# 3dlg-hcvc/tricolo

Hardware: AMD Instinct MI355X
Metric: trimodal training samples/sec (32^3 voxel + 6-view) (higher is better)
Workload: dtype f16 (f16 activation storage + f16 MFMA operands, fp32 accumulate; bf16x3 heads/GRU; within 1e-3 of the fp32 reference)

## Files before the change

### include/tricolo_hip.h

```cpp
#ifndef TRICOLO_HIP_H
#define TRICOLO_HIP_H
#include <stddef.h>
#include <stdint.h>

#ifdef __cplusplus
extern "C" {
#endif

#define TRI_FMT_F32 0
#define TRI_FMT_BF16 1
#define TRI_FMT_F16 2

int tri_version(void);
const char* tri_last_error(void);

typedef struct TriConvDesc {
    int B, ID, IH, IW, Cin;
    int OD, OH, OW, Cout;
    int KD, KH, KW, stride, pad_d, pad_h, pad_w;
} TriConvDesc;

int tri_conv_kpad(int ntaps, int cin_stored);
typedef struct TriPrepDesc {
    const float* w;
// ... 16 lines not shown
int tri_linear_small_supported(int M, int K, int N);
int tri_linear_small_fwd(const float* x, const float* w, const float* bias, float* y, int M, int K, int N, int act, int split3, void* stream);
int tri_linear_small_dgrad(const float* dout, const float* y, const float* w, float* dx, int M, int K, int N, int act, int split3,
                           void* stream);
int tri_linear_small_wgrad(const float* x, const float* dout, const float* y, float* dw, float* db , int M, int K, int N,
                           int act, int split3, void* stream);
int tri_linear_small_bwd(const float* x, const float* dout, const float* y, const float* w, float* dx, float* dw, float* db, int M, int K,
                         int N, int act, int split3, void* stream);

int tri_conv_num_mtiles(const TriConvDesc* d, int split3);
int tri_conv_num_records(const TriConvDesc* d, int split3, int row_list);
int tri_conv_kernel_family(const TriConvDesc* d, int transposed, int split3);
int tri_conv_wgrad_kernel_family(const TriConvDesc* d, int act_fmt);
size_t tri_conv_workspace(const TriConvDesc* d, int transposed);
int tri_conv_fwd(const TriConvDesc* d, const void* in, const void* w_hi, const void* w_lo, void* out, const uint8_t* row_mask,
                 const float* bias, int act, int accumulate, float* stats, int act_fmt, void* workspace, size_t workspace_bytes,
                 const int* row_pos , const int* row_count ,
                 void* stream);
int tri_conv_dgrad(const TriConvDesc* d, const void* dout, const void* wt_hi, const void* wt_lo, void* din, const uint8_t* row_mask,
                   int accumulate, int act_fmt, void* workspace, size_t workspace_bytes,
                   const int* row_pos ,
                   const int* row_count ,
                   void* stream);
typedef struct TriConvBnSums {
    const void* y;
    const float* relu_scale;
    const float* relu_shift;
    const void* relu_out;
    float* partial;
} TriConvBnSums;
int tri_conv_dgrad_bn_records(const TriConvDesc* d, int accumulate, int act_fmt);
int tri_conv_dgrad_bn(const TriConvDesc* d, const void* dout, const void* wt_hi, const void* wt_lo, void* din, int accumulate,
                      int act_fmt, void* workspace, size_t workspace_bytes, const int* row_pos, const TriConvBnSums* sums, void* stream);
size_t tri_conv_wgrad_workspace(const TriConvDesc* d);
size_t tri_conv_plan_bytes(const TriConvDesc* d);
int tri_conv_plan_build(const TriConvDesc* d, void* plan, void* stream);
int tri_conv_wgrad(const TriConvDesc* d, const void* in, const void* dout, const uint8_t* row_mask, const void* plan ,
                   void* workspace, size_t workspace_bytes, float* dw, long s_co, long s_tap, long s_ci, int cin_real, int split3,
                   int act_fmt, float out_scale ,
                   const int* row_pos, const int* row_count ,
                   void* stream);
#ifndef TRI_WGRAD_GROUP_MAX
#define TRI_WGRAD_GROUP_MAX 24
#endif
typedef struct TriWgradReduce {
    const float* slab;
    float* dw;
    long s_co, s_tap, s_ci;
    int splits, Cout, Kpad, ntaps, cin_stored, cin_real, zlanes, nblocks;
    float out_scale;
    int kw_real;
    int kw_shift;
} TriWgradReduce;
int tri_conv_wgrad_partial(const TriConvDesc* d, const void* in, const void* dout, const uint8_t* row_mask, const void* plan ,
                           void* workspace, size_t workspace_bytes, float* dw, long s_co, long s_tap, long s_ci, int cin_real, int split3,
                           int act_fmt, float out_scale, const int* row_pos, const int* row_count, TriWgradReduce* pending ,
                           void* stream);
int tri_wgrad_reduce_grouped(const TriWgradReduce* pending , int n, void* stream);
int tri_wgrad_reduce_grouped_noted(const TriWgradReduce* pending , int n, int* note, void* stream);
#define TRI_WGRAD_JOBS_MAX 12
typedef struct TriWgradJob {
    const TriConvDesc* d;
    const void* in;
    const void* dout;
    const void* plan;
    void* workspace;
// ... 181 lines not shown
```

### tricolo_amd/_C.py

```python
from __future__ import annotations

import ctypes as C
import os

import torch

_HERE = os.path.dirname(os.path.abspath(__file__))
LIB_PATH = os.path.join(_HERE, "libtricolo_hip.so")


class TriConvDesc(C.Structure):
    _fields_ = [(n, C.c_int) for n in ("B", "ID", "IH", "IW", "Cin", "OD", "OH", "OW", "Cout",
                                       "KD", "KH", "KW", "stride", "pad_d", "pad_h", "pad_w")]


class TriPrepDesc(C.Structure):
    _fields_ = [("w", C.c_void_p), ("hi", C.c_void_p), ("lo", C.c_void_p), ("s_row", C.c_long), ("s_tap", C.c_long),
                ("s_inner", C.c_long), ("rows", C.c_int), ("ntaps", C.c_int), ("inner", C.c_int), ("inner_pad", C.c_int),
                ("kpad", C.c_int), ("fmt", C.c_int), ("frag", C.c_int)]


class TriWgradReduce(C.Structure):
    _fields_ = [("slab", C.c_void_p), ("dw", C.c_void_p), ("s_co", C.c_long), ("s_tap", C.c_long), ("s_ci", C.c_long)] + \
               [(n, C.c_int) for n in ("splits", "Cout", "Kpad", "ntaps", "cin_stored", "cin_real", "zlanes", "nblocks")] + \
# ... 9 lines not shown
class TriConvBnSums(C.Structure):
    _fields_ = [("y", C.c_void_p), ("relu_scale", C.c_void_p), ("relu_shift", C.c_void_p), ("relu_out", C.c_void_p), ("partial", C.c_void_p)]


TRI_WGRAD_JOBS_MAX = 12
TRI_ERR_ARG, TRI_ERR_UNSUPPORTED = -1, -2

P, I, L, F, Z, DBL = C.c_void_p, C.c_int, C.c_long, C.c_float, C.c_size_t, C.c_double
DP = C.POINTER(TriConvDesc)

SIGNATURES = {
    "tri_version": (I, []),
    "tri_last_error": (C.c_char_p, []),
    "tri_conv_kpad": (I, [I, I]),
    "tri_weight_prep": (I, [P, L, L, L, I, I, I, I, P, P, I, I, P]),
    "tri_weight_prep_multi": (I, [P, I, P]),
    "tri_embedding_fwd": (I, [P, P, I, I, I, P, P]),
    "tri_embedding_bwd": (I, [P, P, I, I, I, I, I, P, P]),
    "tri_retrieval_topk": (I, [P, P, P, I, I, I, I, P, P, P, P]),
    "tri_linear_small_supported": (I, [I, I, I]),
    "tri_linear_small_fwd": (I, [P, P, P, P, I, I, I, I, I, P]),
    "tri_linear_small_dgrad": (I, [P, P, P, P, I, I, I, I, I, P]),
    "tri_linear_small_wgrad": (I, [P, P, P, P, P, I, I, I, I, I, P]),
    "tri_linear_small_bwd": (I, [P, P, P, P, P, P, P, I, I, I, I, I, P]),
    "tri_conv_num_mtiles": (I, [DP, I]),
    "tri_conv_num_records": (I, [DP, I, I]),
    "tri_conv_workspace": (Z, [DP, I]),
    "tri_conv_kernel_family": (I, [DP, I, I]),
    "tri_conv_wgrad_kernel_family": (I, [DP, I]),
    "tri_conv_fwd": (I, [DP, P, P, P, P, P, P, I, I, P, I, P, Z, P, P, P]),
    "tri_conv_dgrad": (I, [DP, P, P, P, P, P, I, I, P, Z, P, P, P]),
    "tri_conv_dgrad_bn_records": (I, [DP, I, I]),
    "tri_conv_dgrad_bn": (I, [DP, P, P, P, P, I, I, P, Z, P, C.POINTER(TriConvBnSums), P]),
    "tri_conv_wgrad_workspace": (Z, [DP]),
    "tri_conv_plan_bytes": (Z, [DP]),
    "tri_conv_plan_build": (I, [DP, P, P]),
    "tri_conv_wgrad": (I, [DP, P, P, P, P, P, Z, P, L, L, L, I, I, I, F, P, P, P]),
    "tri_conv_wgrad_partial": (I, [DP, P, P, P, P, P, Z, P, L, L, L, I, I, I, F, P, P, P, P]),
    "tri_wgrad_reduce_grouped": (I, [P, I, P]),
    "tri_wgrad_reduce_grouped_noted": (I, [P, I, P, P]),
    "tri_conv_stem_wgrad_bn": (I, [DP, P, P, P, P, P, P, P, P, P, P, Z, P, L, L, L, I, I, F, P, P]),
    "tri_conv_wgrad_group_info": (I, [DP, I, P, P, P]),
    "tri_conv_wgrad_partial_group": (I, [P, I, I, P, P]),
    "tri_bn_finalize": (I, [P, I, I, P, I, P, P, P, P, P, F, F, P, P, P, P, P]),
    "tri_bn_eval_coeffs": (I, [I, P, P, P, P, F, P, P, P, P, P]),
    "tri_bn_act": (I, [P, P, P, P, P, P, P, L, I, I, I, P]),
    "tri_relu_bwd": (I, [P, P, P, L, I, P]),
    "tri_bn_bwd_num_blocks": (I, [L]),
    "tri_bn_bwd_reduce": (I, [P, P, L, I, P, P, P, P, P, I, P]),
    "tri_bn_bwd_finalize": (I, [P, I, I, P, I, P, P, P, P, P, P, P, P, F, P]),
    "tri_bn_bwd_small": (I, [P, P, L, I, P, I, P, P, P, P, P, P, P, P, I, P, P, P, F, I, P]),
    "tri_bn_bwd_apply": (I, [P, P, P, P, P, P, P, L, I, P, P, P, P, I, I, P]),
    "tri_bn_bwd_pair_reduce": (I, [P, P, P, P, L, I, P, P, I, P]),
    "tri_bn_bwd_pair_finalize": (I, [P, P, I, I, I, P, P, P, P, P, P, P, P, F, P]),
    "tri_bn_bwd_pair_apply": (I, [P, P, P, P, P, P, P, P, P, L, I, I, P]),
    "tri_bn_relu_pool3d_fwd": (I, [P, P, P, P, I, I, I, P, P, I, P]),
    "tri_pool3d_bwd_route": (I, [P, P, P, P, P, P, I, I, I, P, I, P]),
    "tri_pool3d_bwd_route_rows": (I, [P, P, P, P, P, P, I, I, I, P, P, P, I, P]),
    "tri_pool3d_bwd_route_rows_num_blocks": (I, [I, I, I]),
    "tri_pool3d_bwd_route_rows_reduce": (I, [P, P, P, P, P, P, I, I, I, P, P, P, P, I, P]),
    "tri_bn_bwd_apply_rows": (I, [P, P, P, P, P, P, I, P, P, L, I, P]),
    "tri_bn_bwd_rows_scratch": (C.c_size_t, [I]),
    "tri_bn_bwd_rows": (I, [P, P, I, P, P, L, P, P, P, P, P, P, F, P, I, P]),
    "tri_pool3d_bwd_route_reduce_num_blocks": (I, [I, I, I]),
    "tri_pool3d_bwd_route_reduce": (I, [P, P, P, P, P, P, I, I, I, P, P, I, P]),
    "tri_maxpool2d_fwd": (I, [P, I, I, I, I, P, P, P, P, I, P]),
# ... 57 lines not shown
    "tri_adam_guard_segments": (I, [P, P, I, L, P, P]),
    "tri_adam_step": (I, [P, P, P, P, L, P, F, P, F, F, F, F, F, P]),
    "tri_adam_step_segments": (I, [P, P, P, I, P, P, L, P, F, P, F, F, F, F, F, P]),
}

_lib = None


def lib():
    global _lib
    if _lib is None:
        if not os.path.exists(LIB_PATH):
            raise ImportError(
                f"{LIB_PATH} not found: the HIP extension is not built.  Run `make -C tricolo_amd/csrc` "
                "(or __graft_entry__.build()).  tricolo_amd has no CPU fallback.")
        l = C.CDLL(LIB_PATH)
        for name, (res, args) in SIGNATURES.items():
            fn = getattr(l, name)
            fn.restype, fn.argtypes = res, args
        _lib = l
    return _lib


class _TimedLib:

    def __init__(self, real):
        self._real, self.records = real, []

    def __getattr__(self, name):
        fn = getattr(self._real, name)
        sig = SIGNATURES.get(name)
        if sig is None or not name.startswith("tri_") or not sig[1] or sig[0] is not I or name in ("tri_last_error",):
            return fn
        if "workspace" in name or "num_" in name or "_info" in name or "kpad" in name or "family" in name or "bytes" in name or "supported" in name or "scratch" in name or "records" in name:
            return fn

        shape_args = {"tri_bn_bwd_reduce": (2, 3), "tri_bn_bwd_apply": (7, 8), "tri_bn_act": (7, 8), "tri_bn_finalize": (1, 2),
                      "tri_bn_bwd_finalize": (1, 2), "tri_bn_bwd_small": (2, 3)}.get(name)

        def timed(*a):
            e0, e1 = torch.cuda.Event(enable_timing=True), torch.cuda.Event(enable_timing=True)
            e0.record()
            rc = fn(*a)
            e1.record()
            key = name if shape_args is None else f"{name}[{int(a[shape_args[0]])}x{int(a[shape_args[1]])}]"
            self.records.append((key, e0, e1))
            return rc
        return timed


def install_timing_proxy():
    global _lib
    real = lib()
    if isinstance(real, _TimedLib):
        return real
    _lib = _TimedLib(real)
    return _lib


def check(rc: int, what: str = ""):
    if rc != 0:
        msg = lib().tri_last_error().decode(errors="replace")
        raise RuntimeError(f"libtricolo_hip {what} failed (code {rc}): {msg}")


def ptr(t):
    if t is None:
# ... 13 lines not shown
```

### tricolo_amd/csrc/conv_igemm.hip

```cpp
#include "common.h"
#include <stdlib.h>
#include <map>
#include <mutex>
#include "../../include/tricolo_hip.h"
#include "conv_vox.h"

struct ConvArgs {
    const void* in;
    const void* w_hi;
    const void* w_lo;
    void* out;
    const uint8_t* row_mask;
    const int* row_pos;
    const int* row_count;
    const float* bias;
    float* stats;
    float* slab;
    int B, ID, IH, IW, Cin;
    int OD, OH, OW, Cout;
    int KD, KH, KW, stride, pd, ph, pw;
    int transposed, act, accumulate;
    int Kpad, M, ntaps, cin_shift, ksplit, steps_per_split;
    unsigned in_bytes;
    int nunits;
    int h_tr, h_rows, h_slab_bytes, h_nr, h_mtiles;
    int h_dbuf;
    int h_abl;
    int h_xcg, h_touch;
    int h_swz;
#ifdef HALO_STAMPS
    long long* h_dbg;
#endif
    FastDiv dOW, dOH, dOD, dCin, dP, dH2;
};

template <int N>
__device__ __forceinline__ float row_ror(float v) {
    return __builtin_bit_cast(float, __builtin_amdgcn_update_dpp(0, __builtin_bit_cast(int, v), 0x120 + N, 0xf, 0xf, false));
}

template <typename AT, int BN, int TM, int TN, int WAVES_M, int WM, int WN>
__device__ __forceinline__ void conv_epilogue(const ConvArgs& p, f32x4 (&acc)[TM][TN], int m0, int n0, int mtile, int wm, int wn, int fr,
                                              int fq, int t, int split, int any_active, float* red, int Meff) {
    if (p.ksplit > 1) {
// ... 282 lines not shown
            }
        };

        if (ks0 < ks1) {
            load_global(ks0);
            store_lds(0);
            __syncthreads();
            for (int ks = ks0; ks < ks1; ++ks) {
                const int buf = (ks - ks0) & 1;
                if (ks + 1 < ks1) load_global(ks + 1);
                compute(buf);
                if (ks + 1 < ks1) store_lds(buf ^ 1);
                __syncthreads();
            }
        }
    }

    conv_epilogue<AT, BN, TM, TN, WAVES_M, WM, WN>(p, acc, m0, n0, mtile, wm, wn, fr, fq, t, split, any_active, red, Meff);
}

__device__ __forceinline__ int dma_off(int row, int chunk) { return row * 128 + (((chunk ^ (row >> 1)) & 7) << 4); }

__device__ __forceinline__ void wait_vmcnt(int n) {
    switch (n) {
#define TRI_W(N) case N: asm volatile("s_waitcnt vmcnt(" #N ")" ::: "memory"); break;
        TRI_W(0) TRI_W(1) TRI_W(2) TRI_W(3) TRI_W(4) TRI_W(5) TRI_W(6) TRI_W(7) TRI_W(8) TRI_W(9) TRI_W(10) TRI_W(11) TRI_W(12)
        TRI_W(13) TRI_W(14) TRI_W(15) TRI_W(16) TRI_W(17) TRI_W(18) TRI_W(19) TRI_W(20) TRI_W(21) TRI_W(22) TRI_W(23) TRI_W(24)
        TRI_W(25) TRI_W(26) TRI_W(27) TRI_W(28) TRI_W(29) TRI_W(30) TRI_W(31) TRI_W(32)
#undef TRI_W
        default: asm volatile("s_waitcnt vmcnt(0)" ::: "memory"); break;
    }
}

template <int BN, int NST, typename AT>
__global__ __launch_bounds__(256) void conv_dma_kernel(const ConvArgs p) {
    typedef Mma<typename OpOf<AT>::E> MM;
    typedef typename MM::v8 v8;
    constexpr int BM = 128, BK = 64;
    constexpr int WAVES_N = 2, WAVES_M = 2;
    constexpr int WM = BM / WAVES_M, WN = BN / WAVES_N, TM = WM / 16, TN = WN / 16;
    constexpr int A_BYTES = BM * 128, B_BYTES = BN * 128, STAGE = A_BYTES + B_BYTES;
    extern __shared__ __attribute__((aligned(16))) char smem[];
    int* lut_off = (int*)(smem + NST * STAGE);
    int* lut_sh = lut_off + 64;
    float* red = (float*)(smem + NST * STAGE + 512);

    const int t = threadIdx.x, lane = t & 63, wave = t >> 6;
    const int NT = p.Cout / BN;
    const int wg = p.row_count ? (int)blockIdx.x : xcd_remap(blockIdx.x, gridDim.x);
    const int mtile = wg / NT, ntile = wg - mtile * NT;
    const int m0 = mtile * BM, n0 = ntile * BN;
    const int sshift = (p.stride == 2) ? 1 : 0;
    const int Meff = p.row_count ? min(*p.row_count, p.M) : p.M;
    if (m0 >= Meff) {
        if (p.stats && p.ksplit == 1 && t < BN) {
            p.stats[((size_t)mtile * 2 + 0) * p.Cout + n0 + t] = 0.f;
            p.stats[((size_t)mtile * 2 + 1) * p.Cout + n0 + t] = 0.f;
        }
        return;
    }

    if (t < 64) {
        int kd = 0, kh = 0, kw = 0;
        if (t < p.ntaps) {
            kw = t % p.KW;
            int r = t / p.KW;
            kh = r % p.KH;
// ... 43 lines not shown
        ax |= (unsigned)__builtin_amdgcn_update_dpp(0, (int)ax, 0x128, 0xf, 0xf, false);
        ax |= (unsigned)__builtin_amdgcn_update_dpp(0, (int)ax, 0x124, 0xf, 0xf, false);
        ax |= (unsigned)__builtin_amdgcn_update_dpp(0, (int)ax, 0x122, 0xf, 0xf, false);
        ax |= (unsigned)__builtin_amdgcn_update_dpp(0, (int)ax, 0x121, 0xf, 0xf, false);
        ax = (unsigned)(__builtin_amdgcn_readlane((int)ax, 0) | __builtin_amdgcn_readlane((int)ax, 16) |
                        __builtin_amdgcn_readlane((int)ax, 32) | __builtin_amdgcn_readlane((int)ax, 48));
        if (lane == 0) wave_axes[wave] = ax;
    }
    any_active = __syncthreads_or(any_active);

    f32x4 acc[TM][TN];
#pragma unroll
    for (int a = 0; a < TM; ++a)
#pragma unroll
        for (int b = 0; b < TN; ++b) acc[a][b] = (f32x4){0.f, 0.f, 0.f, 0.f};

    const int wm = wave / WAVES_N, wn = wave - wm * WAVES_N;
    const int fr = lane & 15, fq = lane >> 4;
    const int split = blockIdx.y;

    if (any_active) {
        const int nk_total = p.Kpad >> 6;
        const int ks0 = split * p.steps_per_split;
        const int ks1 = min(nk_total, ks0 + p.steps_per_split);
        const v4i rsrc = make_rsrc_words(p.in, p.in_bytes);
        const v4i wrsrc = make_rsrc_words((const uint16_t*)p.w_hi + (size_t)n0 * p.Kpad, (unsigned)(BN * p.Kpad * 2));
        const unsigned lds0 = lds_addr(smem) + wave * 1024;
        int woff[BN / 32];
#pragma unroll
        for (int i = 0; i < BN / 32; ++i) {
            int n = (t >> 3) + 32 * i;
            woff[i] = (n * p.Kpad + (slot ^ ((n >> 1) & 7)) * 8) * 2;
        }

        auto issue = [&](int ks, int buf) {
            const unsigned base = lds0 + buf * STAGE;
            const int kb = ks * BK;
            int tap, c0;
            if (p.cin_shift >= 0) { tap = kb >> p.cin_shift; c0 = kb & ((1 << p.cin_shift) - 1); }
            else { tap = (int)fdiv((uint32_t)kb, p.dCin); c0 = kb - tap * p.Cin; }
            const bool tv = tap < p.ntaps;
            const int toff = (lut_off[tv ? tap : 0] + c0) * 2;
            const int sh = lut_sh[tv ? tap : 0];
            const int sx = sh & 255, sy = (sh >> 8) & 255, sz = (sh >> 16) & 255;
#pragma unroll
            for (int i = 0; i < 4; ++i) {
                unsigned mk = rmask[i];
                bool ok = tv && (((mk >> sx) & (mk >> sy) & (mk >> sz)) & 1u);
                int voff = ok ? rowoff[i] + toff : (int)0x80000000;
                dma16_async(rsrc, base + i * 4096, voff);
            }
#pragma unroll
            for (int i = 0; i < BN / 32; ++i) {
                dma16_async(wrsrc, base + A_BYTES + i * 4096, woff[i] + kb * 2);
            }
        };
        auto compute = [&](int buf) {
            const char* base = smem + buf * STAGE;
            const char* bb = base + A_BYTES;
#pragma unroll
            for (int kk = 0; kk < 2; ++kk) {
                v8 ah[TM];
#pragma unroll
                for (int a = 0; a < TM; ++a) ah[a] = *(const v8*)(base + dma_off(wm * WM + a * 16 + fr, kk * 4 + fq));
#pragma unroll
                for (int b = 0; b < TN; ++b) {
                    v8 bhf = *(const v8*)(bb + dma_off(wn * WN + b * 16 + fr, kk * 4 + fq));
#pragma unroll
                    for (int a = 0; a < TM; ++a) acc[a][b] = MM::mma(bhf, ah[a], acc[a][b]);
                }
            }
        };

        int nl = ks1 - ks0;
        if (p.row_pos) {
            if (wave == 0) {
                const unsigned axes = wave_axes[0] | wave_axes[1] | wave_axes[2] | wave_axes[3];
                int count = 0;
                for (int base = 0; base < ks1 - ks0; base += 64) {
                    const int ks = ks0 + base + lane;
                    bool ok = false;
                    if (ks < ks1) {
                        const int kb = ks * BK;
                        const int tap = p.cin_shift >= 0 ? (kb >> p.cin_shift) : (int)fdiv((uint32_t)kb, p.dCin);
                        if (tap < p.ntaps) {
                            const int sh = lut_sh[tap];
                            ok = ((axes >> (sh & 255)) & (axes >> ((sh >> 8) & 255)) & (axes >> ((sh >> 16) & 255))) & 1u;
                        }
                    }
                    const unsigned long long bal = __ballot(ok);
                    if (ok && count + __popcll(bal & ((1ull << lane) - 1ull)) < 256)
                        live_steps[count + __popcll(bal & ((1ull << lane) - 1ull))] = ks;
                    count += __popcll(bal);
                }
                if (lane == 0) nlive_s = count;
            }
            __syncthreads();
            nl = nlive_s;
        }
        auto step_at = [&](int j) { return p.row_pos ? live_steps[j] : ks0 + j; };
        if (nl > 0) {
            constexpr int PER = 4 + BN / 32;
#pragma unroll
            for (int d = 0; d < NST - 1; ++d)
                if (d < nl) issue(step_at(d), d);
            int buf = 0;
            for (int j = 0; j < nl; ++j) {
                const int younger = min(nl - 1 - j, NST - 2);
                if (NST == 2 || younger == 0) wait_vmcnt(0);
                else if (younger == 1) wait_vmcnt(PER);
                else wait_vmcnt(2 * PER);
                __builtin_amdgcn_s_barrier();
                asm volatile("" ::: "memory");
                if (j + NST - 1 < nl) {
                    int nb = buf + NST - 1;
                    if (nb >= NST) nb -= NST;
                    issue(step_at(j + NST - 1), nb);
                }
                compute(buf);
                if (++buf == NST) buf = 0;
            }
        }
        __syncthreads();
    }
    conv_epilogue<AT, BN, TM, TN, WAVES_M, WM, WN>(p, acc, m0, n0, mtile, wm, wn, fr, fq, t, split, any_active, red, Meff);
// ... 1857 lines not shown
    return conv_dispatch(a, act_fmt, workspace, workspace_bytes, (hipStream_t)stream);
}

extern "C" int tri_conv_dgrad_bn_records(const TriConvDesc* d, int accumulate, int act_fmt) {
    (void)accumulate;
    if (act_fmt != TRI_FMT_BF16 && act_fmt != TRI_FMT_F16) return 0;
    ConvPlan pl = conv_make_plan(d->B, d->OD, d->OH, d->OW, d->Cout, d->ID, d->IH, d->IW, d->Cin, d->KD, d->KH, d->KW, d->stride, d->pad_d,
                                 d->pad_h, d->pad_w, 2, 0);
    if (pl.c64 && d->IW <= 32) return pl.c64_grid;
    return 0;
}
extern "C" int tri_conv_dgrad_bn(const TriConvDesc* d, const void* dout, const void* wt_hi, const void* wt_lo, void* din, int accumulate,
                                 int act_fmt, void* workspace, size_t workspace_bytes, const int* row_pos, const TriConvBnSums* sums,
                                 void* stream) {
    if (!sums || !sums->y || !sums->partial || (!sums->relu_scale != !sums->relu_shift) || (sums->relu_scale && sums->relu_out)) {
        tri_set_error("tri_conv_dgrad_bn: sums needs y, partial and at most one of (relu_scale + relu_shift) / relu_out");
        return TRI_ERR_ARG;
    }
    if (tri_conv_dgrad_bn_records(d, accumulate, act_fmt) == 0) {
        tri_set_error("tri_conv_dgrad_bn: no fused form for this layer (tri_conv_dgrad_bn_records == 0)");
        return TRI_ERR_UNSUPPORTED;
    }
    ConvArgs a{};
    a.in = dout; a.w_hi = wt_hi; a.w_lo = wt_lo; a.out = din;
    a.row_pos = row_pos;
    a.B = d->B; a.ID = d->OD; a.IH = d->OH; a.IW = d->OW; a.Cin = d->Cout;
    a.OD = d->ID; a.OH = d->IH; a.OW = d->IW; a.Cout = d->Cin;
    a.KD = d->KD; a.KH = d->KH; a.KW = d->KW; a.stride = d->stride; a.pd = d->pad_d; a.ph = d->pad_h; a.pw = d->pad_w;
    a.transposed = 1; a.act = 0; a.accumulate = accumulate;
    a.ntaps = d->KD * d->KH * d->KW;
    a.M = d->B * d->ID * d->IH * d->IW;
    return conv_dispatch(a, act_fmt, workspace, workspace_bytes, (hipStream_t)stream, sums);
}
```

### tricolo_amd/model/module/img_encoder/mv_cnn.py

```python
from __future__ import annotations

import os

import torch
import torch.nn as nn

from .... import ops
from ....layers import SideStream, TriModule, linear_bwd, linear_fwd, require_gpu


_DS_FWD = int(os.environ.get("TRICOLO_DS_FWD", "2"))
_DS_BWD = int(os.environ.get("TRICOLO_DS_BWD", "2"))
_PREP_DGRAD_LATE = os.environ.get("TRICOLO_PREP_DGRAD_LATE", "1") != "0"
_BN_PAIR = True
_STEM_BESIDE_WGRAD = os.environ.get("TRICOLO_STEM_BESIDE_WGRAD", "1") != "0"
_PREP_ISSUE = int(os.environ.get("TRICOLO_PREP_ISSUE", "1"))


class _BasicBlockParams(nn.Module):
    def __init__(self, inplanes, planes, stride):
        super().__init__()
        self.conv1 = nn.Conv2d(inplanes, planes, 3, stride, 1, bias=False)
        self.bn1 = nn.BatchNorm2d(planes)
        self.relu = nn.ReLU(inplace=True)
        self.conv2 = nn.Conv2d(planes, planes, 3, 1, 1, bias=False)
        self.bn2 = nn.BatchNorm2d(planes)
        self.downsample = None
        if stride != 1 or inplanes != planes:
            self.downsample = nn.Sequential(nn.Conv2d(inplanes, planes, 1, stride, bias=False), nn.BatchNorm2d(planes))
        self.stride = stride


def _resnet18_trunk_params():
    layers = [nn.Conv2d(3, 64, 7, 2, 3, bias=False), nn.BatchNorm2d(64), nn.ReLU(inplace=True), nn.MaxPool2d(3, 2, 1)]
    inpl = 64
    for planes, stride in ((64, 1), (128, 2), (256, 2), (512, 2)):
        layers.append(nn.Sequential(_BasicBlockParams(inpl, planes, stride), _BasicBlockParams(planes, planes, 1)))
        inpl = planes
    layers.append(nn.AdaptiveAvgPool2d((1, 1)))
    net = nn.Sequential(*layers)
    for m in net.modules():
        if isinstance(m, nn.Conv2d):
            nn.init.kaiming_normal_(m.weight, mode="fan_out", nonlinearity="relu")
    return net

# ... 230 lines not shown
    def _backward_blocks(self, blocks, saved_blocks, dout, gr, prec, ugs, batch=None):
        side = self._side
        pattern = "m"
        turn = [0]

        def wgrad_async(x, dy, g, w):
            ch = pattern[turn[0] % len(pattern)]
            turn[0] += 1
            if ch == "m":
                gr[w] = ops.conv_wgrad(x, dy, g, w, prec, out_scale=ugs, batch=batch)
                return
            with torch.cuda.stream(side.fork(x, dy)):
                gr[w] = ops.conv_wgrad(x, dy, g, w, prec, out_scale=ugs)

        dout_sums = None
        for bi in range(len(blocks) - 1, -1, -1):
            blk, sv = blocks[bi], saved_blocks[bi]
            x, y1, co1, g1, a1, y2, co2, g2, yd, cod, gd, out = sv
            pair = (_BN_PAIR and blk.downsample is not None and batch is not None and dout_sums is None and yd is not None
                    and yd.shape == y2.shape and ops._sync_world() == 1)
            dyd_pair = None
            if pair:
                (dy2, gr[blk.bn2.weight], gr[blk.bn2.bias], dyd_pair, gr[blk.downsample[1].weight],
                 gr[blk.downsample[1].bias]) = ops.bn_bwd_pair(y2, co2, blk.bn2.weight, yd, cod, blk.downsample[1].weight, dout, out, g2.M,
                                                               g_masked=dout, out_scale=ugs)
            else:
                dy2, gr[blk.bn2.weight], gr[blk.bn2.bias] = ops.bn_bwd(y2, dout, co2, blk.bn2.weight, count_host=g2.M, inplace=False,
                                                                       relu_out=out, g_masked=dout, out_scale=ugs, partial=dout_sums)
            g = dout
            fine = ops.TIMELINE is not None and ops.TIMELINE.get("fine")
            tag = f"image.bwd.c{y2.shape[-1]}.b{bi}"
            if fine:
                ops.stamp(tag + ".bn2")
            mode = _DS_BWD if (blk.downsample is not None and batch is not None) else 0
            ev = None
            if mode == 2:
                ev = torch.cuda.Event()
                ev.record()

            def shortcut_bwd():
                with torch.cuda.stream(self._side_ds.fork(g, yd, event=ev)):
                    if dyd_pair is not None:
                        return dyd_pair, ops.conv_dgrad(dyd_pair, gd, self._packed[(id(blk.downsample[0]), True)])
                    dyd_, gr[blk.downsample[1].weight], gr[blk.downsample[1].bias] = ops.bn_bwd(
                        yd, g, cod, blk.downsample[1].weight, count_host=gd.M, inplace=False, out_scale=ugs)
                    if batch is None:
                        gr[blk.downsample[0].weight] = ops.conv_wgrad(x, dyd_, gd, blk.downsample[0].weight, prec, out_scale=ugs)
                    return dyd_, ops.conv_dgrad(dyd_, gd, self._packed[(id(blk.downsample[0]), True)])
            if blk.downsample is not None and not mode:
                dyd, dx = shortcut_bwd()
            wgrad_async(a1, dy2, g2, blk.conv2.weight)
            da1, sums1 = ops.conv_dgrad(dy2, g2, self._packed[(id(blk.conv2), True)], bn_sums=(y1, co1, None))
            if mode:
                dyd, dx = shortcut_bwd()
            if fine:
                ops.stamp(tag + ".dgrad2")
            dy1, gr[blk.bn1.weight], gr[blk.bn1.bias] = ops.bn_bwd(y1, da1, co1, blk.bn1.weight, count_host=g1.M, relu=True, out_scale=ugs,
                                                                   partial=sums1)
            if fine:
                ops.stamp(tag + ".bn1")
            wgrad_async(x, dy1, g1, blk.conv1.weight)
            if blk.downsample is not None:
                if batch is None:
                    self._side_ds.join(dx, gr[blk.downsample[0].weight], gr[blk.downsample[1].weight], gr[blk.downsample[1].bias])
                else:
                    self._side_ds.join(dx, dyd, gr[blk.downsample[1].weight], gr[blk.downsample[1].bias])
                    gr[blk.downsample[0].weight] = ops.conv_wgrad(x, dyd, gd, blk.downsample[0].weight, prec, out_scale=ugs, batch=batch)
            else:
                dx = g
            if bi > 0:
                prev = saved_blocks[bi - 1]
                dx, dout_sums = ops.conv_dgrad(dy1, g1, self._packed[(id(blk.conv1), True)], out=dx, accumulate=True,
                                               bn_sums=(prev[5], None, prev[11]))
            else:
                dx, dout_sums = ops.conv_dgrad(dy1, g1, self._packed[(id(blk.conv1), True)], out=dx, accumulate=True), None
            if fine:
                ops.stamp(tag + ".dgrad1")
            dout = dx
        side.join(*[v for v in gr.values() if v.dim() == 4])
        return dout

    def _backward_upper(self, saved, dz, batch=None):
        prec, B = self._prec(), saved["B"]
        gr = {}
        ops.stamp("image.bwd.start")
        self._join_packing_dgrad()
        own = batch is None
        if own:
            batch = ops.wgrad_batch(dz.device)
        do = ops.l2norm_bwd(saved["z"], saved["norm"], dz)
        dh, gr[self.mlp[2].weight], gr[self.mlp[2].bias] = linear_bwd(saved["h"], self.mlp[2].weight, saved["o"], do, 0, prec)
        df, gr[self.mlp[0].weight], gr[self.mlp[0].bias] = linear_bwd(saved["f"], self.mlp[0].weight, saved["h"], dh, 1, prec)
        dp, gr[self.net_2.weight], gr[self.net_2.bias] = linear_bwd(saved["pooled"], self.net_2.weight, saved["f"], df, 0, prec)
        gs = ops.grad_scale(prec)
        dout = ops.avgpool_viewmax_bwd(dp, saved["arg"], saved["feat_shape"], B, self.num_views, dtype=ops.act_dtype(prec), scale=gs)
        ops.stamp("image.bwd.heads.end")
        dx2 = self._backward_blocks(self._blocks()[self.N_LOWER_BLOCKS:], saved["blocks"], dout, gr, prec, 1.0 / gs, batch)
        ops.stamp("image.bwd.layer3.end")
        if own and batch is not None:
            batch.flush()
        return dx2, [gr[p] for p in self._upper_params()]

    def _backward_lower(self, saved, dout, batch=None, stem_side=None):
        prec = self._prec()
        ugs = 1.0 / ops.grad_scale(prec)
        gr = {}
        self._join_packing_dgrad()
        own = batch is None
# ... 101 lines not shown
```

### tricolo_amd/ops.py

```python
from __future__ import annotations

import math
import os

import torch

from . import _C
from ._C import check, lib, make_desc, ptr, stream

_PRECISIONS = ("bf16", "bf16x3", "f16")
_FMT = {torch.float32: 0, torch.bfloat16: 1, torch.float16: 2}
F16_GRAD_SCALE = float(os.environ.get("TRICOLO_F16_GRAD_SCALE", "4096"))
if not (F16_GRAD_SCALE >= 1.0 and math.frexp(F16_GRAD_SCALE)[0] == 0.5):
    raise ValueError(f"TRICOLO_F16_GRAD_SCALE={F16_GRAD_SCALE!r}: must be a power of two >= 1 (the kernels divide it out exactly)")
_default_precision = os.environ.get("TRICOLO_PRECISION", "bf16x3")


def set_default_precision(p: str):
    global _default_precision
    if p not in _PRECISIONS:
        raise ValueError(f"precision must be one of {_PRECISIONS}")
    _default_precision = p


# ... 302 lines not shown
        if tab is None or tab[3] != tuple(w.data_ptr() for (w, _, _) in self.entries.values()):
            tab = self._build(precision, device)
            self._tables[precision] = tab
        raw, n, bufs, _ = tab
        check(lib().tri_weight_prep_multi(ptr(raw), n, stream()), "tri_weight_prep_multi")
        return bufs


def conv_fwd(x, g: ConvGeom, packed, row_mask=None, bias=None, act=0, want_stats=False, out=None, accumulate=False, rows=None):
    hi, lo = packed
    g.check_packed(packed, False, x)
    OD, OH, OW = g.out_grid
    if out is None:
        out = torch.empty((g.B, OD, OH, OW, g.cout), dtype=x.dtype, device=x.device)
    assert out.dtype == x.dtype
    nrec = (g.num_records_rows if rows else g.num_mtiles)[_conv_mode(x, lo)]
    stats = torch.empty((nrec, 2, g.cout), dtype=torch.float32, device=x.device) if want_stats else None
    ws = _workspace(g.fwd_ws, x.device) if g.fwd_ws else None
    check(_timed(_igemm_symbol(g, False, lo is not None, x), _flops(g, rows, row_mask),
                 lambda: lib().tri_conv_fwd(_C.C.byref(g.desc), ptr(_act(x)), ptr(hi), ptr(lo), ptr(out), ptr(row_mask), ptr(bias),
                                            act, 1 if accumulate else 0, ptr(stats), _abf(x), ptr(ws),
                                            ws.numel() if ws is not None else 0, ptr(rows[0]) if rows else None,
                                            ptr(rows[1]) if rows else None, stream())), "tri_conv_fwd")
    return (out, stats) if want_stats else out


_ROW_ORDER = True


_DGRAD_BN_MODE = os.environ.get("TRICOLO_DGRAD_BN", "2")
_DGRAD_BN = _DGRAD_BN_MODE != "0"


def conv_dgrad(dout, g: ConvGeom, packed_t, row_mask=None, out=None, accumulate=False, rows=None, bn_sums=None):
    hi, lo = packed_t
    g.check_packed(packed_t, True, dout)
    ID, IH, IW = g.in_grid
    if out is None:
        out = torch.empty((g.B, ID, IH, IW, g.cin_stored), dtype=dout.dtype, device=dout.device)
    assert out.dtype == dout.dtype
    ws = _workspace(g.dgrad_ws, dout.device) if g.dgrad_ws else None
    rowpos = g.dgrad_row_order(dout.device) if (row_mask is None and rows is None and _ROW_ORDER) else None
    if rows is not None:
        rowpos = rows[0]
    if bn_sums is not None:
        y, co, relu_out = bn_sums
        nrec = g.dgrad_bn_records(accumulate, _abf(dout)) if (_DGRAD_BN and not (accumulate and _DGRAD_BN_MODE == "2") and row_mask is None and rows is None and lo is None
                                                               and (relu_out is not None) == bool(accumulate)
                                                               and (co is not None) != (relu_out is not None)) else 0
        if nrec == 0:
            return conv_dgrad(dout, g, packed_t, row_mask=row_mask, out=out, accumulate=accumulate, rows=rows), None
        assert y.dtype == out.dtype and y.numel() == out.numel()
        partial = torch.empty((nrec, 2, g.cin_stored), dtype=torch.float32, device=dout.device)
        sums = _C.TriConvBnSums(ptr(y), ptr(co.scale) if co is not None else None, ptr(co.shift) if co is not None else None,
                                ptr(relu_out), ptr(partial))
        check(_timed(_igemm_symbol(g, True, False, dout), g.flops,
                     lambda: lib().tri_conv_dgrad_bn(_C.C.byref(g.desc), ptr(_act(dout)), ptr(hi), None, ptr(out), 1 if accumulate else 0,
                                                     _abf(dout), ptr(ws), ws.numel() if ws is not None else 0, ptr(rowpos),
                                                     _C.C.byref(sums), stream())), "tri_conv_dgrad_bn")
        return out, partial
    check(_timed(_igemm_symbol(g, True, lo is not None, dout), _flops(g, rows, row_mask),
                 lambda: lib().tri_conv_dgrad(_C.C.byref(g.desc), ptr(_act(dout)), ptr(hi), ptr(lo), ptr(out), ptr(row_mask),
                                              1 if accumulate else 0, _abf(dout), ptr(ws), ws.numel() if ws is not None else 0,
                                              ptr(rowpos), ptr(rows[1]) if rows else None, stream())), "tri_conv_dgrad")
    return out


_wgrad_ws = {}


def _workspace(nbytes: int, device) -> torch.Tensor:
    key = (device, torch.cuda.current_stream().cuda_stream)
    ws = _wgrad_ws.get(key)
# ... 1131 lines not shown
```

Before: 13200.

## Fuse downsample shortcut dgrad into the 3x3 stride-2 conv dgrad kernel

Adds a shortcut variant of the DMA implicit-GEMM conv kernel that appends the 1x1 stride-2 downsample convolution's dgrad as extra K-steps at the centre tap. The multi-view CNN backward pass uses it by default for eligible residual blocks. This removes the separate shortcut dgrad launch and the accumulate read-modify-write of dx. In exchange, the shortcut work is no longer overlapped on a side stream, and the bn_sums fusion of the preceding block's dgrad is skipped for fused blocks.

After: 13220, median of 2. About the same (+0.1%).

```diff
diff --git a/include/tricolo_hip.h b/include/tricolo_hip.h
--- a/include/tricolo_hip.h
+++ b/include/tricolo_hip.h
@@ -72,6 +72,9 @@
 int tri_conv_dgrad_bn_records(const TriConvDesc* d, int accumulate, int act_fmt);
 int tri_conv_dgrad_bn(const TriConvDesc* d, const void* dout, const void* wt_hi, const void* wt_lo, void* din, int accumulate,
                       int act_fmt, void* workspace, size_t workspace_bytes, const int* row_pos, const TriConvBnSums* sums, void* stream);
+int tri_conv_dgrad_shortcut_ok(const TriConvDesc* d, const TriConvDesc* d2, int act_fmt);
+int tri_conv_dgrad_shortcut(const TriConvDesc* d, const TriConvDesc* d2, const void* dout, const void* dout2, const void* wt, const void* wt2,
+                            void* din, int act_fmt, void* workspace, size_t workspace_bytes, const int* row_pos, void* stream);
 size_t tri_conv_wgrad_workspace(const TriConvDesc* d);
 size_t tri_conv_plan_bytes(const TriConvDesc* d);
 int tri_conv_plan_build(const TriConvDesc* d, void* plan, void* stream);
diff --git a/tricolo_amd/_C.py b/tricolo_amd/_C.py
--- a/tricolo_amd/_C.py
+++ b/tricolo_amd/_C.py
@@ -65,6 +65,8 @@
     "tri_conv_dgrad": (I, [DP, P, P, P, P, P, I, I, P, Z, P, P, P]),
     "tri_conv_dgrad_bn_records": (I, [DP, I, I]),
     "tri_conv_dgrad_bn": (I, [DP, P, P, P, P, I, I, P, Z, P, C.POINTER(TriConvBnSums), P]),
+    "tri_conv_dgrad_shortcut_ok": (I, [DP, DP, I]),
+    "tri_conv_dgrad_shortcut": (I, [DP, DP, P, P, P, P, P, I, P, Z, P, P]),
     "tri_conv_wgrad_workspace": (Z, [DP]),
     "tri_conv_plan_bytes": (Z, [DP]),
     "tri_conv_plan_build": (I, [DP, P, P]),
@@ -188,7 +190,7 @@
         sig = SIGNATURES.get(name)
         if sig is None or not name.startswith("tri_") or not sig[1] or sig[0] is not I or name in ("tri_last_error",):
             return fn
-        if "workspace" in name or "num_" in name or "_info" in name or "kpad" in name or "family" in name or "bytes" in name or "supported" in name or "scratch" in name or "records" in name:
+        if "workspace" in name or "num_" in name or "_info" in name or "kpad" in name or "family" in name or "bytes" in name or "supported" in name or "scratch" in name or "records" in name or name.endswith("_ok"):
             return fn
 
         shape_args = {"tri_bn_bwd_reduce": (2, 3), "tri_bn_bwd_apply": (7, 8), "tri_bn_act": (7, 8), "tri_bn_finalize": (1, 2),
diff --git a/tricolo_amd/csrc/conv_igemm.hip b/tricolo_amd/csrc/conv_igemm.hip
--- a/tricolo_amd/csrc/conv_igemm.hip
+++ b/tricolo_amd/csrc/conv_igemm.hip
@@ -10,6 +10,8 @@
     const void* w_hi;
     const void* w_lo;
     void* out;
+    const void* in2;
+    const void* w2;
     const uint8_t* row_mask;
     const int* row_pos;
     const int* row_count;
@@ -358,7 +360,7 @@
     }
 }
 
-template <int BN, int NST, typename AT>
+template <int BN, int NST, typename AT, bool SC = false>
 __global__ __launch_bounds__(256) void conv_dma_kernel(const ConvArgs p) {
     typedef Mma<typename OpOf<AT>::E> MM;
     typedef typename MM::v8 v8;
@@ -468,8 +470,34 @@
             int n = (t >> 3) + 32 * i;
             woff[i] = (n * p.Kpad + (slot ^ ((n >> 1) & 7)) * 8) * 2;
         }
-
+        const int nk2 = SC ? (p.Cin >> 6) : 0;
+        const int sc_tap = p.ntaps >> 1;
+        v4i rsrc2 = rsrc, wrsrc2 = wrsrc;
+        if (SC) {
+            rsrc2 = make_rsrc_words(p.in2, p.in_bytes);
+            wrsrc2 = make_rsrc_words((const uint16_t*)p.w2 + (size_t)n0 * p.Cin, (unsigned)(BN * p.Cin * 2));
+        }
+
+        auto issue_shortcut = [&](int ks, int buf) {
+            const unsigned base = lds0 + buf * STAGE;
+            const int c0 = (ks - nk_total) * BK;
+            const int sh = lut_sh[sc_tap];
+            const int sx = sh & 255, sy = (sh >> 8) & 255, sz = (sh >> 16) & 255;
+#pragma unroll
+            for (int i = 0; i < 4; ++i) {
+                unsigned mk = rmask[i];
+                bool ok = ((mk >> sx) & (mk >> sy) & (mk >> sz)) & 1u;
+                int voff = ok ? rowoff[i] + c0 * 2 : (int)0x80000000;
+                dma16_async(rsrc2, base + i * 4096, voff);
+            }
+#pragma unroll
+            for (int i = 0; i < BN / 32; ++i) {
+                int n = (t >> 3) + 32 * i;
+                dma16_async(wrsrc2, base + A_BYTES + i * 4096, (n * p.Cin + (slot ^ ((n >> 1) & 7)) * 8 + c0) * 2);
+            }
+        };
         auto issue = [&](int ks, int buf) {
+            if (SC && ks >= nk_total) { issue_shortcut(ks, buf); return; }
             const unsigned base = lds0 + buf * STAGE;
             const int kb = ks * BK;
             int tap, c0;
@@ -508,7 +536,7 @@
             }
         };
 
-        int nl = ks1 - ks0;
+        int nl = ks1 - ks0 + nk2;
         if (p.row_pos) {
             if (wave == 0) {
                 const unsigned axes = wave_axes[0] | wave_axes[1] | wave_axes[2] | wave_axes[3];
@@ -527,6 +555,13 @@
                     const unsigned long long bal = __ballot(ok);
                     if (ok && count + __popcll(bal & ((1ull << lane) - 1ull)) < 256)
                         live_steps[count + __popcll(bal & ((1ull << lane) - 1ull))] = ks;
+                    count += __popcll(bal);
+                }
+                if (SC) {
+                    const int sh = lut_sh[sc_tap];
+                    const bool ok = lane < nk2 && (((axes >> (sh & 255)) & (axes >> ((sh >> 8) & 255)) & (axes >> ((sh >> 16) & 255))) & 1u);
+                    const unsigned long long bal = __ballot(ok);
+                    if (ok && count + lane < 256) live_steps[count + lane] = nk_total + lane;
                     count += __popcll(bal);
                 }
                 if (lane == 0) nlive_s = count;
@@ -2450,3 +2485,70 @@
     a.M = d->B * d->ID * d->IH * d->IW;
     return conv_dispatch(a, act_fmt, workspace, workspace_bytes, (hipStream_t)stream, sums);
 }
+
+template <int NST, typename AT>
+static int launch_dma_shortcut(const ConvArgs& a, hipStream_t stream) {
+    constexpr int BN = 64;
+    constexpr size_t smem = NST * (128 * 128 + BN * 128) + 512 + (size_t)4 * BN * 2 * sizeof(float);
+    static bool attr = false;
+    if (!attr) {
+        hipFuncSetAttribute((const void*)conv_dma_kernel<BN, NST, AT, true>, hipFuncAttributeMaxDynamicSharedMemorySize, (int)smem);
+        attr = true;
+    }
+    conv_dma_kernel<BN, NST, AT, true><<<dim3(((a.M + 127) / 128) * (a.Cout / BN), 1), 256, smem, stream>>>(a);
+    return tri_check_launch("tri_conv_dgrad_shortcut");
+}
+
+static const char* dgrad_shortcut_refusal(const TriConvDesc* d, const TriConvDesc* d2, int act_fmt) {
+    if (!d || !d2) return "both layer descriptors are required";
+    if (act_fmt != TRI_FMT_BF16 && act_fmt != TRI_FMT_F16) return "16-bit activation storage only";
+    if (d->KD != 1 || d->KH != 3 || d->KW != 3 || d->stride != 2 || d->pad_d != 0 || d->pad_h != 1 || d->pad_w != 1 || d->ID != 1 || d->OD != 1)
+        return "the opening layer must be a 2D 3x3 / 2 / pad 1 convolution";
+    if (d2->KD != 1 || d2->KH != 1 || d2->KW != 1 || d2->stride != 2 || d2->pad_d != 0 || d2->pad_h != 0 || d2->pad_w != 0 || d2->ID != 1 || d2->OD != 1)
+        return "the shortcut must be a 2D 1x1 / 2 / pad 0 convolution";
+    if (d->B != d2->B || d->Cin != d2->Cin || d->Cout != d2->Cout || d->IH != d2->IH || d->IW != d2->IW || d->OH != d2->OH || d->OW != d2->OW)
+        return "the two layers differ in batch, channels or image size";
+    if (d->B < 1 || d->IH < 2 || d->IW < 2 || (d->IH & 1) || (d->IW & 1) || d->OH != d->IH / 2 || d->OW != d->IW / 2)
+        return "input sizes must be even (output = input / 2)";
+    if (d->Cin % 64 != 0 || d->Cout % 64 != 0) return "channel counts must be multiples of 64";
+    if ((size_t)d->B * d->OH * d->OW * d->Cout * 2 >= ((size_t)1 << 31) || (size_t)d->B * d->IH * d->IW * d->Cin * 2 >= ((size_t)1 << 31))
+        return "tensor >= 2 GiB (32-bit buffer offsets)";
+    if (10 * d->Cout / 64 > 256) return "more than 256 k-steps (the live-step table of conv_dma_kernel)";
+    if (dma_disabled()) return "conv_dma_kernel is switched off (TRICOLO_NO_DMA)";
+    return nullptr;
+}
+
+extern "C" int tri_conv_dgrad_shortcut_ok(const TriConvDesc* d, const TriConvDesc* d2, int act_fmt) {
+    return dgrad_shortcut_refusal(d, d2, act_fmt) == nullptr ? 1 : 0;
+}
+
+extern "C" int tri_conv_dgrad_shortcut(const TriConvDesc* d, const TriConvDesc* d2, const void* dout, const void* dout2, const void* wt,
+                                       const void* wt2, void* din, int act_fmt, void* workspace, size_t workspace_bytes, const int* row_pos,
+                                       void* stream) {
+    (void)workspace; (void)workspace_bytes;
+    if (const char* why = dgrad_shortcut_refusal(d, d2, act_fmt)) {
+        static thread_local char msg[256];
+        snprintf(msg, sizeof msg, "tri_conv_dgrad_shortcut: %s", why);
+        tri_set_error(msg);
+        return TRI_ERR_ARG;
+    }
+    if (!dout || !dout2 || !wt || !wt2 || !din) { tri_set_error("tri_conv_dgrad_shortcut: dout, dout2, wt, wt2 and din are required"); return TRI_ERR_ARG; }
+    ConvArgs a{};
+    a.in = dout; a.w_hi = wt; a.in2 = dout2; a.w2 = wt2; a.out = din;
+    a.row_pos = row_pos;
+    a.B = d->B; a.ID = 1; a.IH = d->OH; a.IW = d->OW; a.Cin = d->Cout;
+    a.OD = 1; a.OH = d->IH; a.OW = d->IW; a.Cout = d->Cin;
+    a.KD = 1; a.KH = 3; a.KW = 3; a.stride = 2; a.pd = 0; a.ph = 1; a.pw = 1;
+    a.transposed = 1; a.act = 0; a.accumulate = 0;
+    a.ntaps = 9;
+    a.M = d->B * d->IH * d->IW;
+    a.Kpad = 9 * a.Cin;
+    a.cin_shift = ilog2_exact(a.Cin);
+    a.in_bytes = (unsigned)((size_t)a.B * a.IH * a.IW * a.Cin * 2);
+    a.ksplit = 1; a.nunits = a.Kpad / 64; a.steps_per_split = a.nunits;
+    a.dOW = make_fastdiv(a.OW); a.dOH = make_fastdiv(a.OH); a.dOD = make_fastdiv(a.OD); a.dCin = make_fastdiv(a.Cin);
+    const int nst = dma_stages_for(a, 64) >= 3 ? 3 : 2;
+    hipStream_t s = (hipStream_t)stream;
+    if (act_fmt == TRI_FMT_F16) return nst == 3 ? launch_dma_shortcut<3, f16_t>(a, s) : launch_dma_shortcut<2, f16_t>(a, s);
+    return nst == 3 ? launch_dma_shortcut<3, bf16_t>(a, s) : launch_dma_shortcut<2, bf16_t>(a, s);
+}
diff --git a/tricolo_amd/model/module/img_encoder/mv_cnn.py b/tricolo_amd/model/module/img_encoder/mv_cnn.py
--- a/tricolo_amd/model/module/img_encoder/mv_cnn.py
+++ b/tricolo_amd/model/module/img_encoder/mv_cnn.py
@@ -11,6 +11,7 @@
 
 _DS_FWD = int(os.environ.get("TRICOLO_DS_FWD", "2"))
 _DS_BWD = int(os.environ.get("TRICOLO_DS_BWD", "2"))
+_DS_FUSED = int(os.environ.get("TRICOLO_DS_FUSED", "1"))
 _PREP_DGRAD_LATE = os.environ.get("TRICOLO_PREP_DGRAD_LATE", "1") != "0"
 _BN_PAIR = True
 _STEM_BESIDE_WGRAD = os.environ.get("TRICOLO_STEM_BESIDE_WGRAD", "1") != "0"
@@ -307,7 +308,10 @@
             tag = f"image.bwd.c{y2.shape[-1]}.b{bi}"
             if fine:
                 ops.stamp(tag + ".bn2")
-            mode = _DS_BWD if (blk.downsample is not None and batch is not None) else 0
+            packed1 = self._packed[(id(blk.conv1), True)]
+            fused = (dyd_pair is not None and _DS_FUSED and packed1[1] is None and ops.dgrad_shortcut_ok(g1, gd, dyd_pair.dtype)
+                     and (_DS_FUSED != 2 or (g1.kernel_family[(True, 2)] & 255) == 2))
+            mode = _DS_BWD if (blk.downsample is not None and batch is not None and not fused) else 0
             ev = None
             if mode == 2:
                 ev = torch.cuda.Event()
@@ -322,7 +326,7 @@
                     if batch is None:
                         gr[blk.downsample[0].weight] = ops.conv_wgrad(x, dyd_, gd, blk.downsample[0].weight, prec, out_scale=ugs)
                     return dyd_, ops.conv_dgrad(dyd_, gd, self._packed[(id(blk.downsample[0]), True)])
-            if blk.downsample is not None and not mode:
+            if blk.downsample is not None and not mode and not fused:
                 dyd, dx = shortcut_bwd()
             wgrad_async(a1, dy2, g2, blk.conv2.weight)
             da1, sums1 = ops.conv_dgrad(dy2, g2, self._packed[(id(blk.conv2), True)], bn_sums=(y1, co1, None))
@@ -335,6 +339,13 @@
             if fine:
                 ops.stamp(tag + ".bn1")
             wgrad_async(x, dy1, g1, blk.conv1.weight)
+            if fused:
+                gr[blk.downsample[0].weight] = ops.conv_wgrad(x, dyd_pair, gd, blk.downsample[0].weight, prec, out_scale=ugs, batch=batch)
+                dx, dout_sums = ops.conv_dgrad(dy1, g1, packed1, shortcut=(dyd_pair, gd, self._packed[(id(blk.downsample[0]), True)])), None
+                if fine:
+                    ops.stamp(tag + ".dgrad1")
+                dout = dx
+                continue
             if blk.downsample is not None:
                 if batch is None:
                     self._side_ds.join(dx, gr[blk.downsample[0].weight], gr[blk.downsample[1].weight], gr[blk.downsample[1].bias])
@@ -345,10 +356,9 @@
                 dx = g
             if bi > 0:
                 prev = saved_blocks[bi - 1]
-                dx, dout_sums = ops.conv_dgrad(dy1, g1, self._packed[(id(blk.conv1), True)], out=dx, accumulate=True,
-                                               bn_sums=(prev[5], None, prev[11]))
+                dx, dout_sums = ops.conv_dgrad(dy1, g1, packed1, out=dx, accumulate=True, bn_sums=(prev[5], None, prev[11]))
             else:
-                dx, dout_sums = ops.conv_dgrad(dy1, g1, self._packed[(id(blk.conv1), True)], out=dx, accumulate=True), None
+                dx, dout_sums = ops.conv_dgrad(dy1, g1, packed1, out=dx, accumulate=True), None
             if fine:
                 ops.stamp(tag + ".dgrad1")
             dout = dx
diff --git a/tricolo_amd/ops.py b/tricolo_amd/ops.py
--- a/tricolo_amd/ops.py
+++ b/tricolo_amd/ops.py
@@ -358,13 +358,34 @@
 _DGRAD_BN = _DGRAD_BN_MODE != "0"
 
 
-def conv_dgrad(dout, g: ConvGeom, packed_t, row_mask=None, out=None, accumulate=False, rows=None, bn_sums=None):
+def dgrad_shortcut_ok(g: ConvGeom, gd: ConvGeom, dtype) -> bool:
+    c = g.__dict__.setdefault("_dgrad_shortcut", {})
+    k = (id(gd), dtype)
+    if k not in c:
+        c[k] = (gd, dtype in (torch.bfloat16, torch.float16) and g.cin == g.cin_stored and
+                bool(lib().tri_conv_dgrad_shortcut_ok(_C.C.byref(g.desc), _C.C.byref(gd.desc), _FMT[dtype])))
+    return c[k][1]
+
+
+def conv_dgrad(dout, g: ConvGeom, packed_t, row_mask=None, out=None, accumulate=False, rows=None, bn_sums=None, shortcut=None):
     hi, lo = packed_t
     g.check_packed(packed_t, True, dout)
     ID, IH, IW = g.in_grid
     if out is None:
         out = torch.empty((g.B, ID, IH, IW, g.cin_stored), dtype=dout.dtype, device=dout.device)
     assert out.dtype == dout.dtype
+    if shortcut is not None:
+        dyd, gd, packed_d = shortcut
+        if accumulate or row_mask is not None or rows is not None or lo is not None or packed_d[1] is not None:
+            raise RuntimeError("conv_dgrad: the shortcut form stores its result and takes no row mask / list or split operands")
+        gd.check_packed(packed_d, True, dyd)
+        assert dyd.dtype == dout.dtype and dyd.shape == dout.shape
+        check(_timed(f"conv_dma_kernel<64, {_TNAME[dout.dtype]}, shortcut>", g.flops + gd.flops,
+                     lambda: lib().tri_conv_dgrad_shortcut(_C.C.byref(g.desc), _C.C.byref(gd.desc), ptr(_act(dout)), ptr(_act(dyd)), ptr(hi),
+                                                           ptr(packed_d[0]), ptr(out), _abf(dout), None, 0,
+                                                           ptr(g.dgrad_row_order(dout.device)) if _ROW_ORDER else None, stream())),
+              "tri_conv_dgrad_shortcut")
+        return (out, None) if bn_sums is not None else out
     ws = _workspace(g.dgrad_ws, dout.device) if g.dgrad_ws else None
     rowpos = g.dgrad_row_order(dout.device) if (row_mask is None and rows is None and _ROW_ORDER) else None
     if rows is not None:
```
